# malani86/unet-DC-segmentation

Measured on AMD Instinct MI355X. Metric: images/sec fwd+bwd, 512x512x1 U-Net-DC, bs=8/GPU, higher is better.
Workload: dtype bf16

## Files before the change

unet_dc_segmentation_amd/build.py:

```python
from __future__ import annotations

import os
import shutil
import subprocess
import sys

HERE = os.path.dirname(os.path.abspath(__file__))
CSRC = os.path.join(HERE, "csrc")
SOURCES = ["abi.hip", "igemm_conv.hip", "igemm_dma.hip", "igemm_dma16.hip", "igemm_halo.hip", "igemm_lattice.hip", "wgrad.hip", "wgrad_dma.hip", "wgrad_fused.hip", "wgrad_rect.hip", "convt_wgrad.hip", "first_conv.hip", "first_conv_mfma.hip", "partials.hip", "batchnorm.hip", "head.hip", "pack.hip", "loss.hip", "optim.hip", "ccl.hip", "split.hip", "shape.hip", "confidence.hip", "hull.hip", "outlines.hip", "polyfill.hip", "match.hip", "neighbors.hip", "spatial.hip", "boundary.hip", "diffmap.hip", "clean.hip", "sweep.hip", "tile.hip", "tta.hip", "preprocess.hip", "window.hip", "augment.hip", "crop.hip", "density.hip", "border.hip"]
HEADERS = ["common.h", "kernels.h", "workspace.h", "partials.h", "bn_bwd_terms.h", "ccl_uf.h", "pair_table.h", "wave_ops.h", "lds_dma.h", "wgrad_frag.h", "igemm_epilogue.h", "igemm_epilogue16.h", "gather_index.h", "linear_u8.h", "hash32.h", os.path.join("..", "..", "include", "unetdc_hip.h")]
OUT = os.path.join(HERE, "libunetdc_hip.so")


def _hipcc():
    for cand in (shutil.which("hipcc"), "/opt/rocm/bin/hipcc"):
        if cand and os.path.exists(cand):
            return cand
    raise RuntimeError("hipcc not found (ROCm toolchain required to build the gfx950 kernels)")


def needs_build():
    if not os.path.exists(OUT):
        return True
    t = os.path.getmtime(OUT)
    deps = [os.path.join(CSRC, f) for f in SOURCES + HEADERS]
    return any(os.path.getmtime(d) > t for d in deps)


FLAGS = ["--offload-arch=gfx950", "-O3", "-std=c++17", "-fPIC", "-Wall", "-Wno-unused-function", "-fno-slp-vectorize"]
OBJ_DIR = os.path.join(CSRC, "_obj")


def _includes(path, seen=None):
    import re
    seen = set() if seen is None else seen
    for m in re.finditer(r'^\s*#include\s+"([^"]+)"', open(path).read(), re.M):
        q = os.path.normpath(os.path.join(os.path.dirname(path), m.group(1)))
        if q not in seen and os.path.exists(q):
            seen.add(q)
            _includes(q, seen)
    return seen


def _object_key(src):
    import hashlib
    h = hashlib.sha256(" ".join(FLAGS).encode())
    for q in [src] + sorted(_includes(src)):
        h.update(open(q, "rb").read())
    return h.hexdigest()[:16]


def build(force=False, verbose=True):
    if not force and not needs_build():
        return OUT
    from concurrent.futures import ThreadPoolExecutor
    os.makedirs(OBJ_DIR, exist_ok=True)
    hipcc = _hipcc()

    def one(f):
        src = os.path.join(CSRC, f)
        obj = os.path.join(OBJ_DIR, f"{os.path.splitext(f)[0]}.{_object_key(src)}.o")
        if force or not os.path.exists(obj):
            for old in os.listdir(OBJ_DIR):
                if old.startswith(os.path.splitext(f)[0] + "."):
                    os.unlink(os.path.join(OBJ_DIR, old))
            cmd = [hipcc, *FLAGS, "-c", src, "-o", obj]
            if verbose:
                print("[unetdc build]", " ".join(cmd), flush=True)
            r = subprocess.run(cmd, capture_output=True, text=True)
            if r.returncode != 0:
                sys.stderr.write(r.stdout + r.stderr)
                raise RuntimeError(f"hipcc failed on {f}")
        return obj

    with ThreadPoolExecutor(max_workers=min(8, os.cpu_count() or 1)) as ex:
        objs = list(ex.map(one, SOURCES))
    cmd = [hipcc, "--offload-arch=gfx950", "-shared", "-fPIC", *objs, "-o", OUT]
    r = subprocess.run(cmd, capture_output=True, text=True)
    if r.returncode != 0:
        sys.stderr.write(r.stdout + r.stderr)
        raise RuntimeError("hipcc failed linking libunetdc_hip.so")
    return OUT


def _objdump():
    for cand in (shutil.which("llvm-objdump"), "/opt/rocm/lib/llvm/bin/llvm-objdump"):
        if cand and os.path.exists(cand):
            return cand
    raise RuntimeError("llvm-objdump not found")


def device_code_objects(so_path=OUT):
    import struct
    data = open(so_path, "rb").read()
    magic, pos, out = b"__CLANG_OFFLOAD_BUNDLE__", 0, []
    while True:
        i = data.find(magic, pos)
        if i < 0:
            return out
        n, = struct.unpack_from("<Q", data, i + 24)
        q = i + 32
        for _ in range(n):
            off, size, idl = struct.unpack_from("<QQQ", data, q)
            q += 24
            tid = data[q:q + idl].decode()
            q += idl
            if "gfx950" in tid and size:
                out.append(data[i + off:i + off + size])
        pos = i + 24


def packed_f32_report(so_path=OUT):
    import re
    import tempfile
    rep = {}
    for k, elf in enumerate(device_code_objects(so_path)):
        with tempfile.NamedTemporaryFile(suffix=".co") as f:
            f.write(elf)
            f.flush()
            r = subprocess.run([_objdump(), "-d", "--no-show-raw-insn", f.name], capture_output=True, text=True)
        if r.returncode != 0:
            raise RuntimeError("llvm-objdump failed: " + r.stderr[:300])
        cur = None
        for line in r.stdout.splitlines():
            m = re.match(r"^[0-9a-f]+ <(\S+)>:", line)
            if m:
                cur = m.group(1)
                rep.setdefault(cur, 0)
            elif cur and re.search(r"\bv_pk_(add|mul|fma)_f32\b", line):
                rep[cur] += 1
    return rep


if __name__ == "__main__":
    build(force="--force" in sys.argv)
```

unet_dc_segmentation_amd/csrc/igemm_conv.hip:

```cpp
#include <stdlib.h>

#include <stdio.h>

#include "kernels.h"

namespace unetdc {

template <typename T> struct Mma;
template <> struct Mma<bf16_t> {
  __device__ static __forceinline__ void run(f32x16& acc, const u32x4& a, const u32x4& b) {
    acc = __builtin_amdgcn_mfma_f32_32x32x16_bf16(__builtin_bit_cast(bf16x8, a), __builtin_bit_cast(bf16x8, b),
                                                  acc, 0, 0, 0);
  }
};
template <> struct Mma<float> {
  __device__ static __forceinline__ void run(f32x16& acc, const u32x4& a, const u32x4& b) {
#pragma unroll
    for (int s = 0; s < 4; ++s) {
      const unsigned int ua = a[s], ub = b[s];
      acc = __builtin_amdgcn_mfma_f32_32x32x2f32(bits_f32(ua), bits_f32(ub), acc, 0, 0, 0);
    }
  }
};

template <typename T> __device__ __forceinline__ void store_pair(T* dst, float v0, float v1);
template <> __device__ __forceinline__ void store_pair<float>(float* dst, float v0, float v1) {
  *reinterpret_cast<float2*>(dst) = make_float2(v0, v1);
}
template <> __device__ __forceinline__ void store_pair<bf16_t>(bf16_t* dst, float v0, float v1) {
  bf16_t lo = (bf16_t)v0, hi = (bf16_t)v1;
  *reinterpret_cast<unsigned int*>(dst) = (unsigned int)__builtin_bit_cast(unsigned short, lo) |
                                          ((unsigned int)__builtin_bit_cast(unsigned short, hi) << 16);
}

template <typename T, int WM, int WN>
__global__ __launch_bounds__(256, 2) void igemm_conv_kernel(const IgemmParams p) {
  constexpr int BM = 64 * WM, BN = 64 * WN;
  constexpr int AI = BM / 32, BI = BN / 32;
  constexpr int KE = 128 / (int)sizeof(T);
  constexpr int EPC = 16 / (int)sizeof(T);
  constexpr int STAGE = (BM + BN) * 128;
  extern __shared__ __attribute__((aligned(16))) unsigned char smem[];

  const int tid = threadIdx.x, lane = tid & 63, wave = tid >> 6;
  const int wm = wave / WN, wn = wave % WN;
  const int tile = xcd_remap(blockIdx.x, gridDim.x);
  const int mblk = tile / p.nblocks, nblk = tile - mblk * p.nblocks;
  const int m0 = mblk * BM, n0 = nblk * BN;
  const int c = tid & 7, r0 = tid >> 3;
  const T* __restrict__ xg = reinterpret_cast<const T*>(p.x);
  const T* __restrict__ wg = reinterpret_cast<const T*>(p.w);

  int pix[AI], ys[AI], xs[AI];
  unsigned tapmask = 0;
  const int HoWo = p.Ho * p.Wo;
#pragma unroll
  for (int i = 0; i < AI; ++i) {
    const int m = m0 + r0 + 32 * i;
    if (m < p.M) {
      const int n = m / HoWo, rem = m - n * HoWo;
      const int oy = rem / p.Wo, ox = rem - oy * p.Wo;
      ys[i] = oy * p.stride;
      xs[i] = ox * p.stride;
      pix[i] = (n * p.Hi + ys[i]) * p.Wi + xs[i];
    } else {
      ys[i] = -(1 << 28);
      xs[i] = 0;
      pix[i] = 0;
    }
    for (int t = 0; t < p.ntaps; ++t) {
      const int iy = ys[i] + p.offy[t], ix = xs[i] + p.offx[t];
      if ((unsigned)iy < (unsigned)p.Hi && (unsigned)ix < (unsigned)p.Wi) tapmask |= 1u << t;
    }
  }
  {
    unsigned* sm_u = reinterpret_cast<unsigned*>(smem);
    if (tid == 0) sm_u[0] = 0;
    __syncthreads();
    if (tapmask) atomicOr(&sm_u[0], tapmask);
    __syncthreads();
    tapmask = sm_u[0];
    __syncthreads();
  }
  const int nkc = p.Cin / KE;
  const int nsteps = __popc(tapmask) * nkc;

  const int swz_w = (r0 >> 1) & 7;
  int a_wr[AI], b_wr[BI];
#pragma unroll
  for (int i = 0; i < AI; ++i) a_wr[i] = (r0 + 32 * i) * 128 + ((c ^ swz_w) << 4);
#pragma unroll
  for (int i = 0; i < BI; ++i) {
    const int row = r0 + 32 * i, grp = row >> 6, cc = row & 63;
    const int lrow = grp * 64 + (cc & 1) * 32 + (cc >> 1);
    b_wr[i] = BM * 128 + lrow * 128 + ((c ^ ((lrow >> 1) & 7)) << 4);
  }
  const int r = lane & 31, h = lane >> 5;
  const int swz_r = (r >> 1) & 7;
  int a_rd[2][4], b_rd[2][4];
#pragma unroll
  for (int t2 = 0; t2 < 2; ++t2)
#pragma unroll
    for (int g = 0; g < 4; ++g) {
      const int ch = ((2 * g + h) ^ swz_r) << 4;
      a_rd[t2][g] = (wm * 64 + t2 * 32 + r) * 128 + ch;
      b_rd[t2][g] = BM * 128 + (wn * 64 + t2 * 32 + r) * 128 + ch;
    }

  f32x16 acc[2][2];
#pragma unroll
  for (int i = 0; i < 2; ++i)
#pragma unroll
    for (int j = 0; j < 2; ++j)
#pragma unroll
      for (int e = 0; e < 16; ++e) acc[i][j][e] = 0.f;

  u32x4 ra[AI], rb[BI];
  int lt = 0, lkc = 0;
  while (lt < p.ntaps && !((tapmask >> lt) & 1u)) ++lt;

  auto gload = [&]() {
    const int dy = p.offy[lt], dx = p.offx[lt];
    const int dpix = dy * p.Wi + dx;
    const int koff = lkc * KE + c * EPC;
#pragma unroll
    for (int i = 0; i < AI; ++i) {
      const int iy = ys[i] + dy, ix = xs[i] + dx;
      const bool ok = (unsigned)iy < (unsigned)p.Hi && (unsigned)ix < (unsigned)p.Wi;
      u32x4 v = {0u, 0u, 0u, 0u};
      if (ok) v = ld16(xg + ((long)(pix[i] + dpix) * p.ldx + koff));
      ra[i] = v;
    }
#pragma unroll
    for (int i = 0; i < BI; ++i)
      rb[i] = ld16(wg + ((long)(lt * p.Cout + n0 + r0 + 32 * i) * p.Cin + koff));
    if (++lkc == nkc) {
      lkc = 0;
      do { ++lt; } while (lt < p.ntaps && !((tapmask >> lt) & 1u));
    }
  };
  auto lds_store = [&](int stage) {
    unsigned char* base = smem + stage * STAGE;
#pragma unroll
    for (int i = 0; i < AI; ++i) st16(base + a_wr[i], ra[i]);
#pragma unroll
    for (int i = 0; i < BI; ++i) st16(base + b_wr[i], rb[i]);
  };

  if (nsteps > 0) {
    gload();
    lds_store(0);
  }
  __syncthreads();
  for (int s = 0; s < nsteps; ++s) {
    const bool more = (s + 1 < nsteps);
    if (more) gload();
    const unsigned char* base = smem + (s & 1) * STAGE;
#pragma unroll
    for (int g = 0; g < 4; ++g) {
      const u32x4 a0 = ld16(base + a_rd[0][g]), a1 = ld16(base + a_rd[1][g]);
      const u32x4 b0 = ld16(base + b_rd[0][g]), b1 = ld16(base + b_rd[1][g]);
      Mma<T>::run(acc[0][0], a0, b0);
      Mma<T>::run(acc[0][1], a0, b1);
      Mma<T>::run(acc[1][0], a1, b0);
      Mma<T>::run(acc[1][1], a1, b1);
    }
    if (more) lds_store((s + 1) & 1);
    __syncthreads();
  }

  const int col = n0 + wn * 64 + 2 * r;
  T* __restrict__ og = reinterpret_cast<T*>(p.out);
  float k0a = 0.f, k0b = 0.f, k1a = 0.f, k1b = 0.f;
  int shuf_ab = 0, shuf_co = col;
  if (p.mode == MODE_AFFINE_RELU) {
    k0a = p.scale[col]; k0b = p.scale[col + 1];
    k1a = p.shift[col]; k1b = p.shift[col + 1];
  } else if (p.mode == MODE_SHUFFLE) {
    shuf_ab = col / p.shuf_c;
    shuf_co = col - shuf_ab * p.shuf_c;
    if (p.bias) { k1a = p.bias[shuf_co]; k1b = p.bias[shuf_co + 1]; }
  } else if (p.bias) {
    k1a = p.bias[col]; k1b = p.bias[col + 1];
  }
  float s0 = 0.f, q0 = 0.f, s1 = 0.f, q1 = 0.f;
#pragma unroll
  for (int mi = 0; mi < 2; ++mi) {
#pragma unroll
    for (int reg = 0; reg < 16; ++reg) {
      const int m = m0 + wm * 64 + mi * 32 + (reg & 3) + 8 * (reg >> 2) + 4 * h;
      if (m >= p.M) continue;
      float v0 = acc[mi][0][reg], v1 = acc[mi][1][reg];
      if (p.mode == MODE_AFFINE_RELU) {
        v0 = fmaxf(fmaf(v0, k0a, k1a), 0.f);
        v1 = fmaxf(fmaf(v1, k0b, k1b), 0.f);
        store_pair<T>(og + (long)m * p.ldo + col, v0, v1);
      } else if (p.mode == MODE_SHUFFLE) {
        v0 += k1a; v1 += k1b;
        const int n = m / HoWo, rem = m - n * HoWo;
        const int oy = rem / p.Wo, ox = rem - oy * p.Wo;
        const long dst = ((long)(n * 2 * p.Ho + 2 * oy + (shuf_ab >> 1)) * (2 * p.Wo) + 2 * ox + (shuf_ab & 1));
        store_pair<T>(og + dst * p.ldo + shuf_co, v0, v1);
      } else {
        v0 += k1a; v1 += k1b;
        store_pair<T>(og + (long)m * p.ldo + col, v0, v1);
        if (p.mode == MODE_STATS) {
          const float t0 = round_through<T>(v0), t1 = round_through<T>(v1);
          s0 += t0; q0 = fmaf(t0, t0, q0);
          s1 += t1; q1 = fmaf(t1, t1, q1);
        }
      }
    }
  }
  if (p.mode == MODE_STATS) {
    s0 += __shfl_xor(s0, 32, 64); q0 += __shfl_xor(q0, 32, 64);
    s1 += __shfl_xor(s1, 32, 64); q1 += __shfl_xor(q1, 32, 64);
    float* red = reinterpret_cast<float*>(smem);
    if (h == 0) {
      red[(wave * 4 + 0) * 32 + r] = s0;
      red[(wave * 4 + 1) * 32 + r] = q0;
      red[(wave * 4 + 2) * 32 + r] = s1;
      red[(wave * 4 + 3) * 32 + r] = q1;
    }
    __syncthreads();
    if (tid < BN) {
      const int wn2 = tid >> 6, c2 = tid & 63, r2 = c2 >> 1, e = c2 & 1;
      float su = 0.f, sq = 0.f;
#pragma unroll
      for (int w2 = 0; w2 < WM; ++w2) {
        su += red[((w2 * WN + wn2) * 4 + e * 2 + 0) * 32 + r2];
        sq += red[((w2 * WN + wn2) * 4 + e * 2 + 1) * 32 + r2];
      }
      p.stats[((long)mblk * 2 + 0) * p.Cout + n0 + tid] = su;
      p.stats[((long)mblk * 2 + 1) * p.Cout + n0 + tid] = sq;
    }
  }
}

int igemm_mblocks(long M, int Cout) { (void)Cout; return ceil_div(M, 256); }

template <typename T, int WM, int WN>
static int launch_cfg(IgemmParams& p, hipStream_t stream) {
  constexpr int BM = 64 * WM, BN = 64 * WN;
  constexpr int LDS = 2 * (BM + BN) * 128;
  if (const int rc_ = ensure_dynamic_lds(reinterpret_cast<const void*>(&igemm_conv_kernel<T, WM, WN>), LDS, "igemm_conv_kernel")) return rc_;
  p.mblocks = ceil_div(p.M, BM);
  p.nblocks = p.Cout / BN;
  const long nwg = (long)p.mblocks * p.nblocks;
  hipLaunchKernelGGL((igemm_conv_kernel<T, WM, WN>), dim3((unsigned)nwg), dim3(256), LDS, stream, p);
  char nm[96];
  snprintf(nm, sizeof(nm), "igemm_conv_kernel<%s, %d, %d>", sizeof(T) == 2 ? "__bf16" : "float", WM, WN);
  note_kernel(nm);
  return check_launch("igemm_conv_kernel");
}

IgemmPlan plan_igemm(const IgemmParams& p, int dtype) {
  IgemmPlan pl{};
  const bool lattice = igemm_lattice_supported(p, dtype);
  if (p.in_scale) {
    if (lattice && p.mode == MODE_STATS && (p.Cout % 128 == 0 || p.Cin <= 256)) {
      pl.route = IGEMM_LATTICE;
      pl.writes_act = p.Cout % 128 == 0 && (long)p.M * p.Cin * 2 < (1L << 32);
    }
    return pl;
  }
  if (lattice) {
    pl.route = IGEMM_LATTICE;
    return pl;
  }
  if (igemm_halo_supported(p, dtype)) {
    pl.route = IGEMM_HALO;
    return pl;
  }
  const long es = dtype == UNETDC_BF16 ? 2 : 4;
  const long HoWo = (long)p.Ho * p.Wo;
  const long xbytes = (p.M / HoWo) * p.Hi * p.Wi * p.ldx * es;
  const long wbytes = (long)p.ntaps * p.Cout * p.Cin * es;
  const long opix = p.mode == MODE_SHUFFLE ? 4L * p.M : (long)p.M;
  const long obytes = opix * p.ldo * es, ybytes = p.mode == MODE_BNBWD ? (long)p.M * p.bn_ldy * es : 0;
  if (!(xbytes < (1L << 31) && wbytes < (1L << 31) && obytes < (1L << 32) && ybytes < (1L << 32) && p.M % HoWo == 0)) {
    pl.route = IGEMM_FIRSTGEN;
    pl.cfg = (p.Cout % 128 == 0) && p.mode != MODE_STATS;
    return pl;
  }
  const long blocks_a = (long)((p.M + 255) / 256) * (p.Cout / 256);
  const bool use_a = p.Cout % 256 == 0 && p.M >= 256 * 64 && blocks_a >= 200;
  const bool use_b = !use_a && p.Cout % 128 == 0;
  pl.route = IGEMM_DMA;
  pl.cfg = use_a ? 1 : (use_b ? 2 : 3);
  if (dtype == UNETDC_BF16 && p.M % 16 == 0 && !(p.mode == MODE_SHUFFLE && p.Wo % 16 != 0)) {
    pl.route = IGEMM_DMA16;
    const long blocks_b = (long)((p.M + 255) / 256) * (p.Cout / 128);
    if (pl.cfg == 2 && p.mode == MODE_SHUFFLE && p.Cout % 256 == 0 && blocks_a >= 200) pl.cfg = 1;
    else if (pl.cfg == 2 && blocks_b >= 100 && blocks_b < 200) pl.cfg = 3;
  }
  return pl;
}

int launch_igemm(IgemmParams& p, int dtype, hipStream_t stream) {
  const int esz = dtype == UNETDC_BF16 ? 2 : 4;
  const int ke = 128 / esz;
  UNETDC_REQUIRE(dtype == UNETDC_F32 || dtype == UNETDC_BF16, "igemm: bad dtype %d", dtype);
  UNETDC_REQUIRE(p.x && p.w && p.out, "igemm: null tensor pointer");
  UNETDC_REQUIRE(p.M > 0 && p.Cin > 0 && p.Cout > 0, "igemm: empty problem");
  UNETDC_REQUIRE(p.Cin % ke == 0, "igemm: Cin=%d must be a multiple of %d for this dtype", p.Cin, ke);
  UNETDC_REQUIRE(p.Cout % 64 == 0, "igemm: Cout=%d must be a multiple of 64", p.Cout);
  UNETDC_REQUIRE(p.ldx % (16 / esz) == 0 && p.ldo % (16 / esz) == 0, "igemm: ld not 16-byte aligned");
  UNETDC_REQUIRE(((uintptr_t)p.x % 16 == 0) && ((uintptr_t)p.w % 16 == 0) && ((uintptr_t)p.out % 16 == 0),
                 "igemm: pointers must be 16-byte aligned");
  UNETDC_REQUIRE(p.ntaps >= 1 && p.ntaps <= 9, "igemm: ntaps out of range");
  UNETDC_REQUIRE((long)p.M < (1L << 31) - 512, "igemm: too many pixels");
  if (p.mode == MODE_SHUFFLE) UNETDC_REQUIRE(p.shuf_c % 64 == 0, "igemm: convT channels must be a multiple of 64");
  if (p.mode == MODE_STATS) UNETDC_REQUIRE(p.stats != nullptr, "igemm: stats buffer missing");
  if (p.mode == MODE_AFFINE_RELU) UNETDC_REQUIRE(p.scale && p.shift, "igemm: scale/shift missing");
  if (p.mode == MODE_BNBWD)
    UNETDC_REQUIRE(p.stats && p.bn_y && p.scale && p.shift && p.bn_mean && p.bn_rstd, "igemm: BN-backward inputs missing");
  {
    const long howo = (long)p.Ho * p.Wo;
    const bool p2 = (p.Wo & (p.Wo - 1)) == 0 && (howo & (howo - 1)) == 0;
    p.wo_shift = p2 ? __builtin_ctz((unsigned)p.Wo) : -1;
    p.howo_shift = p2 ? __builtin_ctzl((unsigned long)howo) : -1;
  }
  const IgemmPlan pl = plan_igemm(p, dtype);
  switch (pl.route) {
    case IGEMM_LATTICE: return launch_igemm_lattice(p, stream);
    case IGEMM_HALO: return launch_igemm_halo(p, dtype, stream);
    case IGEMM_DMA: return launch_igemm_dma(p, pl.cfg, dtype, stream);
    case IGEMM_DMA16: return launch_igemm_dma16(p, pl.cfg, stream);
    case IGEMM_FIRSTGEN:
      if (p.mode == MODE_BNBWD) {
        set_error("igemm: the first-generation kernel has no fused BatchNorm-backward sums");
        return UNETDC_EUNSUPPORTED;
      }
      if (dtype == UNETDC_BF16) return pl.cfg ? launch_cfg<bf16_t, 2, 2>(p, stream) : launch_cfg<bf16_t, 4, 1>(p, stream);
      return pl.cfg ? launch_cfg<float, 2, 2>(p, stream) : launch_cfg<float, 4, 1>(p, stream);
  }
  set_error("igemm: input normalisation asked for a shape / configuration the lattice kernel does not take");
  return UNETDC_EUNSUPPORTED;
}

}
```

unet_dc_segmentation_amd/csrc/kernels.h:

```cpp
#pragma once
#include <algorithm>
#include <type_traits>

#include "common.h"
#include "workspace.h"
#include "../../include/unetdc_hip.h"

namespace unetdc {

enum { MODE_STORE = 0, MODE_STATS = 1, MODE_AFFINE_RELU = 2, MODE_SHUFFLE = 3, MODE_BNBWD = 4 };
#define UNETDC_EUNSUPPORTED (-4)

struct IgemmParams {
  const void* x;
  const void* w;
  void* out;
  const float* bias;
  const float* scale;
  const float* shift;
  float* stats;
  const void* bn_y;
  const float* bn_mean;
  const float* bn_rstd;
  int bn_ldy;
  int M, Ho, Wo, Hi, Wi, Cin, Cout, ldx, ldo, ntaps, stride, mode, shuf_c;
  int mblocks, nblocks;
  int wo_shift, howo_shift;
  int quad_bpr, quad_bpi;
  const float* in_scale;
  const float* in_shift;
  void* act_out;
  int ld_act;
  int offy[9];
  int offx[9];
};
enum IgemmRoute {
  IGEMM_UNSUPPORTED = 0,
  IGEMM_LATTICE,
  IGEMM_HALO,
  IGEMM_DMA,
  IGEMM_DMA16,
  IGEMM_FIRSTGEN,
};
struct IgemmPlan {
  int route;
  int cfg;
  bool writes_act;
};
IgemmPlan plan_igemm(const IgemmParams& p, int dtype);
int launch_igemm(IgemmParams& p, int dtype, hipStream_t stream);
int igemm_mblocks(long M, int Cout);
bool igemm_lattice_supported(const IgemmParams& p, int dtype);
bool igemm_halo_supported(const IgemmParams& p, int dtype);
int launch_igemm_lattice(IgemmParams& p, hipStream_t stream);
int launch_igemm_halo(IgemmParams& p, int dtype, hipStream_t stream);
int launch_igemm_dma(IgemmParams& p, int cfg, int dtype, hipStream_t stream);
int launch_igemm_dma16(IgemmParams& p, int cfg, hipStream_t stream);

struct WgradParams {
  const void* a;
  const void* b;
  float* part;
  int N, H, W, Hb, Wb, CI, CJ, lda, ldb, ntaps, stride;
  int P;
  int chunk;
  int ksplit, itiles, jtiles;
  int adv_y, adv_x;
  int offy[9];
  int offx[9];
  const float* in_scale;
  const float* in_shift;
};
enum WgradRoute {
  WGRAD_UNSUPPORTED = 0,
  WGRAD_CONVT,
  WGRAD_RECT,
  WGRAD_FUSED,
  WGRAD_DMA,
  WGRAD_LEGACY,
};
struct WgradFusedPlan {
  bool supported;
  bool paired;
  bool bnin;
  int pf;
  int ysplit, rows_per_unit, imgs_per_unit, half_lds;
  int threads, nwg;
  int lds, lds_attr;
  int units;
  long workspace;
};
struct WgradPlan {
  int route;
  WgradFusedPlan fused;
  int ksplit;
  int chunk, tw, step;
  int steps_per_half;
  long workspace;
};
WgradPlan plan_wgrad(const WgradParams& p, int dtype);
long wgrad_workspace_bound(int N, int H, int W, int CI, int CJ, int ntaps, int dtype);
int launch_wgrad(WgradParams& p, float* out, void* workspace, long workspace_bytes, int dtype, hipStream_t stream);
bool convt_wgrad_split(int N, int H, int W, int CI, int CJ, int& ksplit, int& steps_per_half);
int launch_convt_wgrad_fused(const WgradParams& w, const WgradPlan& pl, hipStream_t stream);
int wgrad_rect_units(int N, int H, int W, int CI, int CJ, int d);
int launch_wgrad_rect(const WgradParams& w, const WgradPlan& pl, float* out, hipStream_t stream);
WgradFusedPlan plan_wgrad_fused(const WgradParams& w, int dtype);
long wgrad_fused_workspace_bytes(int N, int H, int W, int CI, int CJ, int dtype);
int launch_wgrad_fused(const WgradParams& w, const WgradFusedPlan& pl, int dtype, hipStream_t stream);
int wgrad_dma_tile(int CI, int CJ);
int wgrad_dma_pixel_step(int dtype, int tw);
int launch_wgrad_dma_kernel(WgradParams& p, int tw, int dtype, hipStream_t stream);

struct FirstParams {
  const float* x;
  const float* w;
  const float* bias;
  const float* scale;
  const float* shift;
  void* y;
  float* stats;
  int N, H, W, Cin, Cout, ldy, dil;
};
struct FirstWgradParams {
  const float* x;
  const void* dy;
  float* part;
  int N, H, W, Cin, Cout, lddy, dil;
  const void* bn_y; int bn_ldy;
  const float* bn_scale; const float* bn_shift; const float* bn_mean; const float* bn_rstd; const float* bn_k;
};
struct FirstPlan {
  bool mfma;
  int fwd_blocks;
  bool wgrad_mfma;
  int wgrad_blocks;
  int rows_blocks;
  long workspace;
};
FirstPlan plan_first(long P, int Cin, int Cout);
int launch_first_fwd(FirstParams& p, int dtype, hipStream_t stream);
bool first_wgrad_bn_supported(int N, int H, int W, int Cin, int Cout, int dil, int dtype);
int launch_bn_bwd_coeffs(const float* pre_parts, int pre_nparts, long count, const float* gamma, const float* rstd, float* dgamma,
                         float* dbeta, float* dbias, float* coeffs, int C, hipStream_t stream);
int first_mfma_mblocks(long P);
int first_mfma_wgrad_blocks(long P);
int launch_first_mfma_fwd(FirstParams& p, int blocks, int dtype, hipStream_t stream);
int launch_first_mfma_wgrad(FirstWgradParams& p, int blocks, int dtype, hipStream_t stream);
int launch_first_wgrad(FirstWgradParams& p, float* dw, void* workspace, long workspace_bytes, int dtype,
                       hipStream_t stream);
int launch_first_dgrad(const void* dy, int lddy, const float* w, float* dx, int N, int H, int W, int Cin, int Cout, int dil,
                       int dtype, hipStream_t stream);

struct ApplyParams {
  const void* y; void* a; void* pooled;
  const float* scale; const float* shift;
  int N, H, W, C, ldy, lda, ldp;
};
struct BnBwdParams {
  const void* dskip; const void* dpool; const void* y; void* dy;
  const float* scale; const float* shift; const float* mean; const float* rstd;
  const float* k1; const float* k2; const float* k3;
  float* parts;
  int N, H, W, C, lds, ldp, ldy, lddy;
  const float* head_dprobs; const float* head_probs; const float* head_w;
};
struct HeadParams {
  const void* a; const float* w; const float* b; float* probs;
  const float* dprobs; void* da; float* parts;
  int N, H, W, C, OC, lda, ldda;
  const void* bn_y; const float* bn_scale; const float* bn_shift; const float* bn_mean; const float* bn_rstd;
  float* bn_parts;
  int bn_ldy;
};
constexpr int SPARE_ROWS = 64;
inline long partial_floats(long rows, long L) { return (rows + SPARE_ROWS) * L; }
inline long partial_row_cap(long floats, long L) { return floats / L - SPARE_ROWS; }
inline int chunk_elems(int dtype) { return dtype == UNETDC_BF16 ? 8 : dtype == UNETDC_F32 ? 4 : 0; }
inline int grid_for(long work_items, int per_block, long cap = 8192) {
  return (int)std::min(std::max((work_items + per_block - 1) / per_block, 1L), cap);
}
template <typename T> struct TypeTag { using type = T; };
template <typename F> void dispatch_flags(F&& f) { f(); }
template <typename F, typename... B> void dispatch_flags(F&& f, bool b, B... rest) {
  if (b) dispatch_flags([&](auto... c) { f(std::true_type{}, c...); }, rest...);
  else dispatch_flags([&](auto... c) { f(std::false_type{}, c...); }, rest...);
}
template <typename F, typename... B> void dispatch(int dtype, F&& f, B... flags) {
  if (dtype == UNETDC_BF16) dispatch_flags([&](auto... c) { f(TypeTag<bf16_t>{}, c...); }, flags...);
  else dispatch_flags([&](auto... c) { f(TypeTag<float>{}, c...); }, flags...);
}
struct BnBwdPlan { bool ok; int epc, cpp, seg, nb, ny, apply_nb; long workspace; };
BnBwdPlan plan_bn_bwd(int N, int H, int W, int C, int pooled, int dtype);
struct HeadPlan { bool ok; int epc, cpp, fwd_nb, bwd_nb; long workspace; };
constexpr long HEAD_BWD_MAX_ROWS = 1024;
HeadPlan plan_head(long P, int C, int OC, int dtype, long row_cap);
struct ChannelSumPlan { bool ok; int epc, nb, ny; long workspace; };
ChannelSumPlan plan_channel_sum(long P, int C, int dtype);

int launch_bn_finalize(const float* parts, int nparts, long count, const float* gamma, const float* beta, float eps,
                       float momentum, float* rm, float* rv, float* scale, float* shift, float* mean, float* rstd,
                       int C, hipStream_t stream);
int launch_bn_eval_affine(const float* gamma, const float* beta, const float* rm, const float* rv,
                          const float* conv_bias, float eps, float* scale, float* shift, int C, hipStream_t stream);
int launch_apply(ApplyParams& p, int dtype, hipStream_t stream);
int launch_bn_bwd(BnBwdParams& p, const float* gamma, float* dgamma, float* dbeta, float* dbias, void* workspace,
                  long workspace_bytes, const float* pre_parts, int pre_nparts, int dtype, hipStream_t stream, bool frozen);
int launch_bn_frozen_affine(const float* gamma, const float* beta, const float* rm, const float* rv, float eps, float* scale,
                            float* shift, float* mean, float* rstd, int C, hipStream_t stream);
int launch_bn_bwd_reduce_only(BnBwdParams& p, float* parts, long parts_floats, int* nparts, int dtype, hipStream_t stream);
int launch_head_fwd(HeadParams& p, int dtype, hipStream_t stream);
int launch_head_bwd(HeadParams& p, float* dw, float* db, void* workspace, long workspace_bytes, int dtype,
                    hipStream_t stream, int* bn_nparts, long bn_parts_floats);
int launch_pack_conv3x3(const float* w, void* wf, void* wd, int Co, int Ci, int dtype, hipStream_t stream);
int launch_pack_convT2x2(const float* w, void* wf, void* wd, int Ci, int Co, int dtype, hipStream_t stream);
int launch_pack_many(const void* table_dev, int n, long total, int dtype, hipStream_t stream);
int launch_adam_step(const void* table_dev, int n, long total_blocks, const float* flat_grad, double lr, double beta1,
                     double beta2, double eps, long step, double grad_scale, int dtype, hipStream_t stream);
long grad_norm_workspace_bytes(long n);
int launch_grad_norm(const float* flat_grad, long n, double grad_scale, double max_norm, void* ctl_dev, void* workspace,
                     long workspace_bytes, hipStream_t stream);
int launch_adam_step_ex(const void* table_dev, int n, long total_blocks, const float* flat_grad, double lr, double beta1,
                        double beta2, double eps, long step, double grad_scale, int dtype, const void* ctl_dev,
                        double weight_decay, float* ema_base, const float* m_base, double ema_decay, hipStream_t stream);
int launch_stats_colsum(const float* parts, int nparts, int ctotal, int c0, int c, float* out, hipStream_t stream);
int launch_channel_sum(const void* x, int ldx, float* out, void* workspace, long workspace_bytes, long P, int C,
                       int dtype, hipStream_t stream);

int launch_mask_from_probs(const float* probs, int ph, int pw, float thresh, unsigned char* mask, int oh, int ow,
                           hipStream_t stream);
int launch_mask_from_probs_linear(const float* probs, int ph, int pw, float thresh, unsigned char* mask, int oh, int ow,
                                  const int* xofs, const short* xcoef, const int* yofs, const short* ycoef, hipStream_t stream);
long ccl_workspace_bytes(int h, int w);
long ccl_labels_workspace_bytes(int h, int w);
int launch_ccl(const char* who, const unsigned char* mask, int h, int w, int min_area, void* workspace, long workspace_bytes,
               int* out_count, int* out_area, long long* out_sumy, long long* out_sumx, int* out_root, int* out_label,
               int max_out, hipStream_t stream);
struct CclPlanes {
  unsigned long long *sy, *sx;
  int *L, *area, *blocksum;
};
struct CclWorkspace {
  CclPlanes ccl;
  int* more;
};
Layout<CclWorkspace> ccl_layout(int h, int w, int extra, void* workspace);
void launch_ccl_init(const unsigned char* mask, const CclPlanes& p, int n, hipStream_t stream);
void launch_ccl_finish(const unsigned char* mask, int h, int w, int min_area, const CclPlanes& p, int* out_count,
                       int* out_area, long long* out_sumy, long long* out_sumx, int* out_root, int* rank_of_root, int max_out,
                       hipStream_t stream);
void launch_ccl_label(const unsigned char* mask, const CclPlanes& p, const int* rank_of_root, int min_area, int* label, int n,
                      hipStream_t stream);
void launch_ccl_scan(int* blocksum, int nblocks, int* total, hipStream_t stream);

constexpr int SHAPE_QUANTITIES = 14;
int launch_label_props(const int* label, const unsigned char* gray, int h, int w, long long* out, int max_out,
                       hipStream_t stream);

constexpr int CONF_QUANTITIES = 10, CONF_IMAGE_QUANTITIES = 8;
int launch_label_confidence(const int* label, int max_out, int h, int w, const float* probs, const float* lo, const float* hi,
                            int ph, int pw, float thresh, float band, const unsigned short* table, long long* out,
                            long long* out_image, unsigned char* out_entropy, unsigned char* out_spread, hipStream_t stream);

long label_overlap_workspace_bytes(int h, int w, int max_pairs);
int launch_label_overlap(const int* label_a, int max_a, const int* label_b, int max_b, int h, int w, void* workspace,
                         long workspace_bytes, int* out_count, int* out_a, int* out_b, int* out_n, int max_pairs,
                         hipStream_t stream);

constexpr int HULL_QUANTITIES = 5;
long label_hull_workspace_bytes(int h, int w, int max_out, int max_rows);
int launch_label_hull(const int* label, int max_out, int h, int w, void* workspace, long workspace_bytes, long long* out,
                      int* out_rows, int max_rows, hipStream_t stream);

constexpr int OUTLINE_QUANTITIES = 6;
constexpr int CONTOUR_FIELDS = 5;
long label_outlines_workspace_bytes(int h, int w, int max_out, int max_cracks);
int launch_label_outlines(const int* label, int max_out, int h, int w, int max_len, void* workspace, long workspace_bytes, long long* out,
                          long long* contours, int max_contours, int* vx, int* vy, int max_vertices, int max_cracks, int* needed,
                          hipStream_t stream);

long polygon_fill_workspace_bytes(int h, int w, int n_polys, int n_rings, int n_verts);
int launch_polygon_fill(const int* verts, const int* ring_first, const int* poly_first_ring, const int* poly_label, int n_polys,
                        int n_rings, int n_verts, int h, int w, int* labels_out, void* workspace, long workspace_bytes,
                        hipStream_t stream);
int launch_label_census(const int* label, int h, int w, int n_labels, long long* area, hipStream_t stream);
int launch_label_relabel(int* label, int h, int w, const int* lut, int n_lut, hipStream_t stream);

long label_neighbors_workspace_bytes(int h, int w, int max_label, int max_pairs);
int launch_label_neighbors(const int* label, int max_label, int h, int w, int radius, void* workspace, long workspace_bytes,
                           int* out_count, int* out_a, int* out_b, int* out_d2, int max_pairs, int* out_nn_label,
                           int* out_nn_d2, int* out_degree, int* out_cluster, int* out_cluster_size, hipStream_t stream);

long ripley_workspace_bytes(int h, int w, int max_points, int rmax, int n_sim);
int launch_droplet_points(const int* count, const int* area, const long long* sum_y, const long long* sum_x, int max_points,
                          const unsigned char* window, int h, int w, int* out_py, int* out_px, int* out_info,
                          hipStream_t stream);
int launch_ripley_counts(const int* py, const int* px, const int* n_points, int max_points, const unsigned char* window, int h,
                         int w, int rmax, int n_sim, unsigned seed, void* workspace, long workspace_bytes, int* out_n,
                         long long* out_pairs, long long* out_pairs_all, hipStream_t stream);

long boundary_distances_workspace_bytes(int h, int w);
int launch_boundary_distances(const int* label_a, int max_a, const int* label_b, int max_b, int h, int w, int radius,
                              void* workspace, long workspace_bytes, long long* hist, int* dmax, long long* out_a,
                              long long* out_b, hipStream_t stream);

int launch_edt_sq(const unsigned char* mask, int h, int w, int* out_d2, void* workspace, long workspace_bytes,
                  hipStream_t stream);
void launch_edt_col(const unsigned char* mask, int* g, int h, int w, hipStream_t stream);
long split_workspace_bytes(int h, int w);
int launch_split_stats(const unsigned char* mask, int h, int w, int min_area, int split_depth_half_px, void* workspace,
                       long workspace_bytes, int* out_count, int* out_area, long long* out_sumy, long long* out_sumx,
                       int* out_root, int* out_label, int max_out, hipStream_t stream);

long mask_clean_workspace_bytes(int h, int w);
int launch_mask_clean(const unsigned char* strong, const unsigned char* weak, int h, int w, int max_hole_area, void* workspace,
                      long workspace_bytes, unsigned char* out_mask, int* out_counts, hipStream_t stream);

long diff_regions_workspace_bytes(int h, int w);
int launch_diff_regions(const unsigned char* pred, const unsigned char* gt, int h, int w, int min_area, void* workspace,
                        long workspace_bytes, long long* out_image, int* out_count, int* out_class, int* out_area,
                        long long* out_sumy, long long* out_sumx, int* out_neighbors, int max_out, hipStream_t stream);
int launch_diff_paint(const unsigned char* pred, const unsigned char* gt, const unsigned char* rgb, int h, int w,
                      unsigned char* out_diff, unsigned char* out_overlay, hipStream_t stream);

int launch_thresh_sweep(const float* probs, int n, int ph, int pw, const unsigned char* gt, int oh, int ow, const int* xofs,
                        const short* xcoef, const int* yofs, const short* ycoef, int k, long long* hist, hipStream_t stream);

int launch_tile_gather(const unsigned char* src, int h, int w, int cn, float* tiles, int t, const int* yo, int ny, const int* xo,
                       int nx, int t0, int count, hipStream_t stream);
int launch_tile_blend(const float* tiles, int t, int overlap, const int* yo, int ny, const int* xo, int nx, float* out, int h,
                      int w, hipStream_t stream);

int launch_dihedral_expand(const float* x, int n, int c, int s, int nvar, float* out, hipStream_t stream);
int launch_dihedral_mean(const float* p, int n, int s, int nvar, float* out, hipStream_t stream);
int launch_dihedral_mean_env(const float* p, int n, int s, int nvar, float* out_mean, float* out_lo, float* out_hi,
                             hipStream_t stream);

constexpr int AUG_HFLIP = 1, AUG_VFLIP = 2, AUG_BC = 4;
constexpr int AUG_MAX_SEEDS = 64;
constexpr int AUG_MAX_BATCH = 32;
struct AugRecord {
  int src, flags, k, field;
  float alpha, beta_max;
  int reserved[2];
};
long elastic_fields_workspace_bytes(int n, int h, int w, double sigma);
int launch_elastic_fields(const unsigned* seeds, int n, int h, int w, double sigma, float alpha, float* fields,
                          void* workspace, long workspace_bytes, hipStream_t stream);
int launch_augment_gather(const float* cache_img, const unsigned char* cache_mask, int ncache, int c, int h, int w,
                          const AugRecord* params, int n, const float* fields, int nfields, float* out_img, float* out_mask,
                          hipStream_t stream);

struct CropRecord {
  long long img_off, mask_off;
  int h, w, y0, x0, flags, k, field;
  float alpha, beta_max;
  int t;
};
int launch_crop_gather(const char* who, bool scaled, const unsigned char* images, long images_bytes, const unsigned char* masks,
                       long masks_bytes, int c, int s, const CropRecord* params, int n, const float* fields, int nfields,
                       float* out_img, float* out_mask, hipStream_t stream);

long rolling_ball_workspace_bytes(int h, int w, int cn);
int launch_rolling_ball(const unsigned char* src, unsigned char* dst, int h, int w, int cn, int k, void* workspace,
                        long workspace_bytes, hipStream_t stream);
int launch_resize_linear_chw(const unsigned char* src, int h, int w, int cn, float* dst, int dh, int dw, const int* xofs,
                             const short* xa, const int* yofs, const short* ya, hipStream_t stream);
int launch_morph_rect(const unsigned char* src, unsigned char* dst, int h, int w, int k, bool is_max, hipStream_t stream);

long u16_ranks_workspace_bytes(int h, int w, int c, int nq);
int launch_u16_ranks(const unsigned short* src, int h, int w, int c, const int* ppm, int nq, void* workspace, long workspace_bytes,
                     int* out_value, int* out_below, int* out_equal, hipStream_t stream);
int launch_window_u16_to_u8(const unsigned short* src, int h, int w, int c, const int* levels, unsigned char* dst, int dc,
                            hipStream_t stream);
int launch_planes_max_u16(const unsigned short* src, int planes, int h, int w, unsigned short* dst, hipStream_t stream);

long density_workspace_bytes(int h, int w);
int launch_density_maps(const unsigned char* rgb, const unsigned char* mask, int h, int w, const int* dcount, const int* darea,
                        const long long* dsumy, const long long* dsumx, int dcap, int nb_layers, double sigma,
                        const double* taps, void* workspace, long workspace_bytes, unetdc_density_stats* stats,
                        unsigned char* radial_index, unsigned char* spatial_index, unsigned char* out_blur,
                        unsigned char* out_roi, unsigned char* out_ring, float* out_radial, float* out_spatial,
                        hipStream_t stream);
int launch_density_sqrt(const long long* x, double* out, long n, hipStream_t stream);

long loss_workspace_bytes(int nimg, long hw);
int launch_loss_fwd(const float* p, const float* t, const float* wt, float* loss_out, float* coef, void* workspace,
                    long workspace_bytes, int nimg, long hw, float alpha, float gamma, float ratio, float smooth,
                    hipStream_t stream);
int launch_loss_bwd(const float* p, const float* t, const float* wt, const float* coef, const float* gout, float* dp, int nimg,
                    long hw, float alpha, float gamma, float ratio, hipStream_t stream);

long border_workspace_bytes(int n, int h, int w, int radius);
int launch_border_weights(const float* target, int n, int h, int w, float w0, float sigma, int radius, float* out_weight,
                          int* out_d1, int* out_d2, void* workspace, long workspace_bytes, hipStream_t stream);

}
```

Baseline: 765.2.

## Add persistent weight-resident streaming kernel for small transposed-conv GEMMs

Adds a persistent kernel for the 2x2 transposed-conv forward (pixel-shuffle) and its stride-2 data-gradient for the 128/64 and 256/128 channel shapes. Each block loads its whole weight slice into LDS once, then loops over pixel tiles with double-buffered DMA loads and 16x16x32 MFMAs, fusing the bias/scatter or BN-backward epilogue. The grid is capped near the CU count so weights are reused across many tiles instead of being reloaded per tile. The trade-off is a large LDS footprint that limits occupancy, plus a new routing branch placed ahead of the existing DMA igemm path.

```diff
diff --git a/unet_dc_segmentation_amd/build.py b/unet_dc_segmentation_amd/build.py
--- a/unet_dc_segmentation_amd/build.py
+++ b/unet_dc_segmentation_amd/build.py
@@ -7,7 +7,7 @@
 
 HERE = os.path.dirname(os.path.abspath(__file__))
 CSRC = os.path.join(HERE, "csrc")
-SOURCES = ["abi.hip", "igemm_conv.hip", "igemm_dma.hip", "igemm_dma16.hip", "igemm_halo.hip", "igemm_lattice.hip", "wgrad.hip", "wgrad_dma.hip", "wgrad_fused.hip", "wgrad_rect.hip", "convt_wgrad.hip", "first_conv.hip", "first_conv_mfma.hip", "partials.hip", "batchnorm.hip", "head.hip", "pack.hip", "loss.hip", "optim.hip", "ccl.hip", "split.hip", "shape.hip", "confidence.hip", "hull.hip", "outlines.hip", "polyfill.hip", "match.hip", "neighbors.hip", "spatial.hip", "boundary.hip", "diffmap.hip", "clean.hip", "sweep.hip", "tile.hip", "tta.hip", "preprocess.hip", "window.hip", "augment.hip", "crop.hip", "density.hip", "border.hip"]
+SOURCES = ["abi.hip", "igemm_conv.hip", "igemm_dma.hip", "igemm_dma16.hip", "igemm_halo.hip", "igemm_lattice.hip", "convt_stream.hip", "wgrad.hip", "wgrad_dma.hip", "wgrad_fused.hip", "wgrad_rect.hip", "convt_wgrad.hip", "first_conv.hip", "first_conv_mfma.hip", "partials.hip", "batchnorm.hip", "head.hip", "pack.hip", "loss.hip", "optim.hip", "ccl.hip", "split.hip", "shape.hip", "confidence.hip", "hull.hip", "outlines.hip", "polyfill.hip", "match.hip", "neighbors.hip", "spatial.hip", "boundary.hip", "diffmap.hip", "clean.hip", "sweep.hip", "tile.hip", "tta.hip", "preprocess.hip", "window.hip", "augment.hip", "crop.hip", "density.hip", "border.hip"]
 HEADERS = ["common.h", "kernels.h", "workspace.h", "partials.h", "bn_bwd_terms.h", "ccl_uf.h", "pair_table.h", "wave_ops.h", "lds_dma.h", "wgrad_frag.h", "igemm_epilogue.h", "igemm_epilogue16.h", "gather_index.h", "linear_u8.h", "hash32.h", os.path.join("..", "..", "include", "unetdc_hip.h")]
 OUT = os.path.join(HERE, "libunetdc_hip.so")
 
diff --git a/unet_dc_segmentation_amd/csrc/convt_stream.hip b/unet_dc_segmentation_amd/csrc/convt_stream.hip
--- /dev/null
+++ b/unet_dc_segmentation_amd/csrc/convt_stream.hip
@@ -0,0 +1,324 @@
+#include <stdio.h>
+#include <stdlib.h>
+
+#include "igemm_epilogue16.h"
+#include "kernels.h"
+#include "lds_dma.h"
+
+namespace unetdc {
+
+namespace {
+constexpr int CS_BM = 256;
+constexpr int CS_W_BYTES = 64 * 1024;
+constexpr int CS_STAGE = CS_BM * 128;
+constexpr int CS_A_OFF = CS_W_BYTES;
+constexpr int CS_RED_OFF = CS_A_OFF + 2 * CS_STAGE;
+constexpr int CS_TAB_OFF = CS_RED_OFF + 8 * 128 * 4;
+constexpr int CS_LDS = CS_TAB_OFF + CS_BM * 4;
+static_assert(CS_LDS <= 160 * 1024, "LDS image does not fit");
+}
+
+#if defined(__HIP_DEVICE_COMPILE__)
+__device__ __forceinline__ void cs_lds_barrier() {
+  asm volatile("s_waitcnt lgkmcnt(0)" ::: "memory");
+  raw_barrier();
+}
+#endif
+
+template <int WM, int WN, int TMT, int MODE>
+__global__ __launch_bounds__(512, 2) void convt_stream_kernel(const IgemmParams p, const int ngroups, const int nsl) {
+#if defined(__HIP_DEVICE_COMPILE__)
+  constexpr int NW = 8;
+  constexpr int NB = WN * 64;
+  constexpr int SPT = 512 / NB;
+  constexpr int NT = MODE == MODE_SHUFFLE ? 1 : 4;
+  constexpr int NST = TMT * 4;
+  static_assert(WM * WN == NW && WM * TMT * 16 == CS_BM, "tile/wave mismatch");
+  static_assert(SPT >= 2, "the forward's pixel table is written behind the barrier of step 0 and read behind that of step 1");
+  static_assert(NST <= 63, "vmcnt is a 6-bit counter");
+  extern __shared__ __attribute__((aligned(16))) unsigned char smem[];
+
+  const int tid = threadIdx.x, lane = tid & 63;
+  const int wave = __builtin_amdgcn_readfirstlane(tid >> 6);
+  const int wm = wave / WN, wn = wave % WN;
+  const int G = gridDim.x, b = blockIdx.x;
+  int slice, group;
+  if (G % (8 * nsl) == 0) {
+    const int local = b >> 3;
+    slice = local % nsl;
+    group = (local / nsl) * 8 + (b & 7);
+  } else {
+    slice = b % nsl;
+    group = b / nsl;
+  }
+  const int mtiles = p.mblocks;
+  if (group >= mtiles) return;
+  const int n0 = slice * NB;
+  const int HoWo = p.Ho * p.Wo;
+  const unsigned lds_base = lds_addr_of(smem);
+
+  const unsigned xbytes = (unsigned)(((long)p.M / HoWo) * p.Hi * p.Wi * p.ldx * 2);
+  const unsigned wbytes = (unsigned)((long)NT * p.Cout * p.Cin * 2);
+  const __amdgpu_buffer_rsrc_t xr = __builtin_amdgcn_make_buffer_rsrc(const_cast<void*>(p.x), 0, xbytes, 0x00020000);
+  const __amdgpu_buffer_rsrc_t wr = __builtin_amdgcn_make_buffer_rsrc(const_cast<void*>(p.w), 0, wbytes, 0x00020000);
+
+  const int sub = lane >> 3, pc = lane & 7;
+#pragma unroll
+  for (int j = 0; j < 8; ++j) {
+    const int widx = wave + NW * j;
+    const int ws = widx / (NB / 8), rbk = widx % (NB / 8);
+    const int lrow = rbk * 8 + sub;
+    const int grp = lrow >> 6, q = lrow & 63;
+    const int cc = (q & 15) * 4 + (q >> 4);
+    const int c = pc ^ ((lrow >> 1) & 7);
+    const int tap = ws % NT, kc = ws / NT;
+    const unsigned soff = (unsigned)__builtin_amdgcn_readfirstlane(tap * p.Cout * p.Cin * 2 + kc * 128);
+    lds_dma16(wr, lds_base + ws * (NB * 128) + rbk * 1024, (unsigned)((n0 + grp * 64 + cc) * p.Cin * 2 + c * 16), soff);
+  }
+
+  unsigned abase[4];
+  auto setup_rows = [&](int tile) {
+#pragma unroll
+    for (int j = 0; j < 4; ++j) {
+      const int row = (wave + NW * j) * 8 + sub;
+      const int m = tile * CS_BM + row;
+      const int c = pc ^ ((row >> 1) & 7);
+      if (m < p.M) {
+        int pix = m;
+        if (MODE != MODE_SHUFFLE) {
+          const int n = m / HoWo, rem = m - n * HoWo;
+          const int oy = rem / p.Wo, ox = rem - oy * p.Wo;
+          pix = (n * p.Hi + 2 * oy) * p.Wi + 2 * ox;
+        }
+        abase[j] = (unsigned)(pix * p.ldx * 2 + c * 16);
+      } else {
+        abase[j] = 0x80000000u;
+      }
+    }
+  };
+  auto issue = [&](int cs) {
+    const int tap = cs % NT, kc = cs / NT;
+    const unsigned dbytes = (unsigned)__builtin_amdgcn_readfirstlane(((tap >> 1) * p.Wi + (tap & 1)) * p.ldx * 2 + kc * 128);
+    const unsigned sbase = lds_base + CS_A_OFF + (cs & 1) * CS_STAGE;
+#pragma unroll
+    for (int j = 0; j < 4; ++j) lds_dma16(xr, sbase + (wave + NW * j) * 1024, abase[j], dbytes);
+  };
+
+  const int c16 = lane & 15, rb = lane >> 4;
+  const int swz = (c16 >> 1) & 7;
+  int a_rd[2], b_rd[2];
+#pragma unroll
+  for (int g = 0; g < 2; ++g) {
+    const int ch = ((4 * g + rb) ^ swz) << 4;
+    a_rd[g] = (wm * TMT * 16 + c16) * 128 + ch;
+    b_rd[g] = (wn * 64 + c16) * 128 + ch;
+  }
+
+  const int col = n0 + wn * 64 + 4 * c16;
+  const unsigned ldob = (unsigned)(p.ldo * 2), ldyb = (unsigned)(p.bn_ldy * 2);
+  int ccol = col;
+  unsigned tapoff = 0;
+  if (MODE == MODE_SHUFFLE) {
+    const int ab = col / p.shuf_c;
+    ccol = col - ab * p.shuf_c;
+    tapoff = (unsigned)(((ab >> 1) * 2 * p.Wo + (ab & 1)) * p.ldo * 2 + ccol * 2);
+  }
+  const Epi16Consts kcn = epi16_consts<MODE == MODE_BNBWD ? MODE_BNBWD : MODE_STORE>(p, ccol);
+  const __amdgpu_buffer_rsrc_t orr = whole_buffer(p.out);
+  const __amdgpu_buffer_rsrc_t yrr = whole_buffer(MODE == MODE_BNBWD ? p.bn_y : p.out);
+  unsigned* const table = reinterpret_cast<unsigned*>(smem + CS_TAB_OFF);
+  float* const red = reinterpret_cast<float*>(smem + CS_RED_OFF);
+
+  setup_rows(group);
+  issue(0);
+  auto run_tile = [&](const int ct, const bool drained, auto full_c) {
+    constexpr bool full = decltype(full_c)::value;
+    const int m0 = ct * CS_BM;
+    bool tile_ok[TMT];
+    unsigned voff[TMT], yoff[TMT];
+#pragma unroll
+    for (int i = 0; i < TMT; ++i) {
+      const int pix = m0 + (wm * TMT + i) * 16;
+      tile_ok[i] = pix < p.M;
+      voff[i] = (unsigned)(pix + 4 * rb) * ldob + (unsigned)(col * 2);
+      yoff[i] = (unsigned)(pix + 4 * rb) * ldyb + (unsigned)(col * 2);
+    }
+    f32x4 acc[TMT][4];
+#pragma unroll
+    for (int i = 0; i < TMT; ++i)
+#pragma unroll
+      for (int j = 0; j < 4; ++j)
+#pragma unroll
+        for (int e = 0; e < 4; ++e) acc[i][j][e] = 0.f;
+    u32x2 ypre[TMT][4];
+
+#pragma unroll
+    for (int cs = 0; cs < SPT; ++cs) {
+      if (cs == 0 && !drained) wait_vmcnt<NST>(); else wait_vmcnt<0>();
+      cs_lds_barrier();
+      if (cs + 1 < SPT) {
+        issue(cs + 1);
+      } else if (ct + ngroups < mtiles) {
+        setup_rows(ct + ngroups);
+        issue(0);
+      }
+      if (MODE == MODE_SHUFFLE && cs == 0 && tid < CS_BM) {
+        const int m = m0 + tid;
+        unsigned o = 0;
+        if (m < p.M) {
+          const int n = m / HoWo, rem = m - n * HoWo;
+          const int oy = rem / p.Wo, ox = rem - oy * p.Wo;
+          o = (unsigned)((n * 2 * p.Ho + 2 * oy) * (2 * p.Wo) + 2 * ox) * ldob;
+        }
+        table[tid] = o;
+      }
+      if (MODE == MODE_BNBWD && cs == SPT - 1 && full) {
+#pragma unroll
+        for (int i = 0; i < TMT; ++i)
+#pragma unroll
+          for (int v = 0; v < 4; ++v) ypre[i][v] = __builtin_amdgcn_raw_buffer_load_b64(yrr, yoff[i], (unsigned)v * ldyb, 0);
+      }
+      const unsigned char* abuf = smem + CS_A_OFF + (cs & 1) * CS_STAGE;
+      const unsigned char* wbuf = smem + cs * (NB * 128);
+#pragma unroll
+      for (int g = 0; g < 2; ++g) {
+        u32x4 fb[4];
+#pragma unroll
+        for (int j = 0; j < 4; ++j) fb[j] = ld16(wbuf + b_rd[g] + j * 16 * 128);
+#pragma unroll
+        for (int i = 0; i < TMT; ++i) {
+          const u32x4 fa = ld16(abuf + a_rd[g] + i * 16 * 128);
+#pragma unroll
+          for (int j = 0; j < 4; ++j)
+            acc[i][j] = __builtin_amdgcn_mfma_f32_16x16x32_bf16(__builtin_bit_cast(bf16x8, fa), __builtin_bit_cast(bf16x8, fb[j]),
+                                                                acc[i][j], 0, 0, 0);
+        }
+      }
+    }
+
+    bool all_ok[TMT];
+#pragma unroll
+    for (int i = 0; i < TMT; ++i) all_ok[i] = true;
+    float s4[4] = {0.f, 0.f, 0.f, 0.f}, q4[4] = {0.f, 0.f, 0.f, 0.f};
+    if (MODE == MODE_SHUFFLE) {
+      auto scatter = [&](const bool (&ok)[TMT]) {
+#pragma unroll
+        for (int i = 0; i < TMT; ++i) {
+          if (!ok[i]) continue;
+          const u32x4 o4 = ld16(table + (wm * TMT + i) * 16 + 4 * rb);
+#pragma unroll
+          for (int v = 0; v < 4; ++v) {
+            const unsigned o = o4[v];
+            const u32x2 pk = pack4_bf16(acc[i][0][v] + kcn.k1[0], acc[i][1][v] + kcn.k1[1], acc[i][2][v] + kcn.k1[2],
+                                        acc[i][3][v] + kcn.k1[3]);
+            __builtin_amdgcn_raw_buffer_store_b64(pk, orr, o + tapoff, 0u, 0);
+          }
+        }
+      };
+      if (full) scatter(all_ok); else scatter(tile_ok);
+    } else if (MODE == MODE_BNBWD) {
+      if (full) epilogue16c<MODE_BNBWD, TMT, true>(p, acc, all_ok, voff, ldob, yoff, ldyb, kcn, s4, q4, ypre);
+      else epilogue16c<MODE_BNBWD, TMT>(p, acc, tile_ok, voff, ldob, yoff, ldyb, kcn, s4, q4);
+#pragma unroll
+      for (int k = 0; k < 4; ++k) {
+        s4[k] += __shfl_xor(s4[k], 16, 64); q4[k] += __shfl_xor(q4[k], 16, 64);
+        s4[k] += __shfl_xor(s4[k], 32, 64); q4[k] += __shfl_xor(q4[k], 32, 64);
+      }
+      if (rb == 0) {
+#pragma unroll
+        for (int k = 0; k < 4; ++k) {
+          red[((wave * 4 + k) * 2 + 0) * 16 + c16] = s4[k];
+          red[((wave * 4 + k) * 2 + 1) * 16 + c16] = q4[k];
+        }
+      }
+      cs_lds_barrier();
+      if (tid < NB) {
+        const int wn2 = tid >> 6, cc = tid & 63, c2 = cc >> 2, k = cc & 3;
+        float su = 0.f, sq = 0.f;
+#pragma unroll
+        for (int w2 = 0; w2 < WM; ++w2) {
+          su += red[(((w2 * WN + wn2) * 4 + k) * 2 + 0) * 16 + c2];
+          sq += red[(((w2 * WN + wn2) * 4 + k) * 2 + 1) * 16 + c2];
+        }
+        p.stats[((long)ct * 3 + 0) * p.Cout + n0 + tid] = su;
+        p.stats[((long)ct * 3 + 1) * p.Cout + n0 + tid] = sq;
+        p.stats[((long)ct * 3 + 2) * p.Cout + n0 + tid] = 0.f;
+      }
+    } else {
+      if (full) epilogue16c<MODE_STORE, TMT>(p, acc, all_ok, voff, ldob, yoff, ldyb, kcn, s4, q4);
+      else epilogue16c<MODE_STORE, TMT>(p, acc, tile_ok, voff, ldob, yoff, ldyb, kcn, s4, q4);
+    }
+  };
+  const int full_tiles = p.M / CS_BM;
+  bool drained = true;
+  int ct = group;
+  for (; ct < full_tiles; ct += ngroups) {
+    run_tile(ct, drained, std::true_type{});
+    drained = false;
+  }
+  if (ct < mtiles) run_tile(ct, drained, std::false_type{});
+#endif
+}
+
+bool convt_stream_supported(const IgemmParams& p, int dtype) {
+  if (dtype != UNETDC_BF16 || p.in_scale) return false;
+  const bool fwd = p.mode == MODE_SHUFFLE && p.ntaps == 1 && p.stride == 1;
+  const bool dgrad = (p.mode == MODE_STORE || p.mode == MODE_BNBWD) && p.ntaps == 4 && p.stride == 2 && p.Hi == 2 * p.Ho &&
+                     p.Wi == 2 * p.Wo;
+  if (!fwd && !dgrad) return false;
+  const int cin = fwd ? p.Cin : p.Cout, cout = fwd ? p.shuf_c : p.Cin;
+  if (fwd && p.Cout != 4 * cout) return false;
+  if (!((cin == 128 && cout == 64) || (cin == 256 && cout == 128))) return false;
+  if (p.M % 16 != 0 || p.M < CS_BM / 2) return false;
+  const long HoWo = (long)p.Ho * p.Wo;
+  if (p.M % HoWo != 0) return false;
+  const long xbytes = (p.M / HoWo) * p.Hi * p.Wi * p.ldx * 2;
+  const long obytes = (fwd ? 4L : 1L) * p.M * p.ldo * 2, ybytes = p.mode == MODE_BNBWD ? (long)p.M * p.bn_ldy * 2 : 0;
+  return xbytes < (1L << 31) && obytes < (1L << 32) && ybytes < (1L << 32);
+}
+
+static int convt_stream_grid_cap() {
+  if (const char* e = getenv("UNETDC_CONVT_STREAM_GRID")) {
+    const int v = atoi(e);
+    if (v > 0) return v;
+  }
+  static int cus[64] = {0};
+  int dev = 0;
+  if (hipGetDevice(&dev) != hipSuccess || dev < 0 || dev >= 64) dev = 0;
+  if (cus[dev] == 0) {
+    int n = 0;
+    if (hipDeviceGetAttribute(&n, hipDeviceAttributeMultiprocessorCount, dev) != hipSuccess || n <= 0) n = 256;
+    cus[dev] = n;
+  }
+  return cus[dev];
+}
+
+template <int WM, int WN, int TMT, int MODE>
+static int launch_convt_stream_cfg(IgemmParams& p, const char* name, hipStream_t stream) {
+  constexpr int NB = WN * 64;
+  if (const int rc_ = ensure_dynamic_lds(reinterpret_cast<const void*>(&convt_stream_kernel<WM, WN, TMT, MODE>), CS_LDS, "convt_stream_kernel")) return rc_;
+  UNETDC_REQUIRE((long)p.ntaps * p.Cin * NB == 32768 && p.Cout % NB == 0, "convt_stream: %d x %d does not fill a weight slice", p.ntaps * p.Cin, NB);
+  p.mblocks = ceil_div(p.M, CS_BM);
+  p.nblocks = p.Cout / NB;
+  const int ngroups = std::min(p.mblocks, std::max(1, convt_stream_grid_cap() / p.nblocks));
+  hipLaunchKernelGGL((convt_stream_kernel<WM, WN, TMT, MODE>), dim3((unsigned)(ngroups * p.nblocks)), dim3(512), CS_LDS, stream, p,
+                     ngroups, p.nblocks);
+  note_kernel(name);
+  return check_launch("convt_stream_kernel");
+}
+
+int launch_convt_stream(IgemmParams& p, hipStream_t stream) {
+  const int K = p.ntaps * p.Cin;
+  if (p.mode == MODE_SHUFFLE) {
+    if (K == 128) return launch_convt_stream_cfg<2, 4, 8, MODE_SHUFFLE>(p, "convt_stream_kernel<fwd>", stream);
+    return launch_convt_stream_cfg<4, 2, 4, MODE_SHUFFLE>(p, "convt_stream_kernel<fwd>", stream);
+  }
+  if (p.mode == MODE_BNBWD) {
+    if (K == 256) return launch_convt_stream_cfg<4, 2, 4, MODE_BNBWD>(p, "convt_stream_kernel<dgrad bnstats>", stream);
+    return launch_convt_stream_cfg<8, 1, 2, MODE_BNBWD>(p, "convt_stream_kernel<dgrad bnstats>", stream);
+  }
+  if (K == 256) return launch_convt_stream_cfg<4, 2, 4, MODE_STORE>(p, "convt_stream_kernel<dgrad>", stream);
+  return launch_convt_stream_cfg<8, 1, 2, MODE_STORE>(p, "convt_stream_kernel<dgrad>", stream);
+}
+
+}
diff --git a/unet_dc_segmentation_amd/csrc/igemm_conv.hip b/unet_dc_segmentation_amd/csrc/igemm_conv.hip
--- a/unet_dc_segmentation_amd/csrc/igemm_conv.hip
+++ b/unet_dc_segmentation_amd/csrc/igemm_conv.hip
@@ -283,6 +283,10 @@
     pl.cfg = (p.Cout % 128 == 0) && p.mode != MODE_STATS;
     return pl;
   }
+  if (convt_stream_supported(p, dtype)) {
+    pl.route = IGEMM_CONVT_STREAM;
+    return pl;
+  }
   const long blocks_a = (long)((p.M + 255) / 256) * (p.Cout / 256);
   const bool use_a = p.Cout % 256 == 0 && p.M >= 256 * 64 && blocks_a >= 200;
   const bool use_b = !use_a && p.Cout % 128 == 0;
@@ -327,6 +331,7 @@
     case IGEMM_HALO: return launch_igemm_halo(p, dtype, stream);
     case IGEMM_DMA: return launch_igemm_dma(p, pl.cfg, dtype, stream);
     case IGEMM_DMA16: return launch_igemm_dma16(p, pl.cfg, stream);
+    case IGEMM_CONVT_STREAM: return launch_convt_stream(p, stream);
     case IGEMM_FIRSTGEN:
       if (p.mode == MODE_BNBWD) {
         set_error("igemm: the first-generation kernel has no fused BatchNorm-backward sums");
diff --git a/unet_dc_segmentation_amd/csrc/kernels.h b/unet_dc_segmentation_amd/csrc/kernels.h
--- a/unet_dc_segmentation_amd/csrc/kernels.h
+++ b/unet_dc_segmentation_amd/csrc/kernels.h
@@ -41,6 +41,7 @@
   IGEMM_DMA,
   IGEMM_DMA16,
   IGEMM_FIRSTGEN,
+  IGEMM_CONVT_STREAM,
 };
 struct IgemmPlan {
   int route;
@@ -56,6 +57,8 @@
 int launch_igemm_halo(IgemmParams& p, int dtype, hipStream_t stream);
 int launch_igemm_dma(IgemmParams& p, int cfg, int dtype, hipStream_t stream);
 int launch_igemm_dma16(IgemmParams& p, int cfg, hipStream_t stream);
+bool convt_stream_supported(const IgemmParams& p, int dtype);
+int launch_convt_stream(IgemmParams& p, hipStream_t stream);
 
 struct WgradParams {
   const void* a;
```

After: 763.1. Within noise of the previous version (-0.3%).
